# shubhamchandak94/HARC

Measured on AMD Instinct MI355X. Metric: Mreads/s reorder+encode, 100 bp, higher is better.
Workload: dtype u64 (2-bit packed bases, XOR+popcount)

## Files before the change

harc_amd/csrc/internal.h:

```cpp
#pragma once
#include <hip/hip_runtime.h>
#include <stdint.h>
#include <stdio.h>
#include <string.h>
#include <map>
#include <string>
#include <utility>
#include <vector>
#include "../../include/harc_amd.h"

#define HARC_NONE 0xFFFFFFFFu
#define HARC_MAXW 8
#define HARC_MAXW3 12
#define HARC_MAXK (1u << 20)
#define HARC_LOOK_CHUNKS 16
#ifndef HARC_NSUGG
#define HARC_NSUGG 8
#endif

void harc_set_error(const char *fmt, ...);

#define HIP_TRY(expr)                                                                                          \
    do {                                                                                                       \
        hipError_t _e = (expr);                                                                                \
// ... 67 lines not shown
    std::vector<PoolChunk> pool;
    size_t pool_cur = 0, pool_total = 0;

    uint32_t N = 0;  uint64_t *d_reads = nullptr;
    uint32_t NN = 0; uint64_t *d_nreads3 = nullptr;
    struct InBuf { void *p = nullptr; size_t cap = 0; };
    InBuf own_reads, own_nreads3;
    uint32_t N_own = 0, NN_own = 0;
    uint64_t nrec_own = 0;
    struct HarcComm *comm = nullptr;
    InBuf x_reads, x_nreads3, x_gid, x_ngid;
    uint32_t *d_gid = nullptr, *d_ngid = nullptr;
    int s2_world = 1, s2_rank = 0;
    bool s2_part = false; int s2_e0 = 0, s2_e1 = 0;
    bool replicated = false;
    uint64_t shard_info[8] = { 0, 0, 0, 0, 0, 0, 0, 0 };
    bool have_s1 = false;
    uint32_t M = 0, S = 0;
    uint32_t *d_order = nullptr; uint8_t *d_flag = nullptr, *d_pos = nullptr, *d_rc = nullptr; uint32_t *d_order_s = nullptr;
    uint64_t *d_oreads = nullptr;
    uint64_t *d_sreads = nullptr;
    bool s1_from_files = false;
    bool have_s2 = false;
    uint32_t *d_s2_order = nullptr, *d_s2_orderN = nullptr; size_t n_s2_order = 0, n_s2_orderN = 0;

    struct OutBuf { const uint8_t *ptr = nullptr; size_t len = 0; std::vector<uint8_t> own; };
    std::map<std::pair<int, int>, OutBuf> out;
    struct HostChunk { char *base; size_t size, used; };
    std::vector<HostChunk> harena;
    harc_amd_counters C;
    uint64_t digest[4] = { 0, 0, 0, 0 }; bool have_digest = false;

    char *feed_ring = nullptr; size_t feed_ring_bytes = 0;

    void *d_tmp = nullptr; size_t tmp_bytes = 0;
};

struct HarcComm {
    int world = 1, rank = 0;
    virtual ~HarcComm() {}
    virtual int allgather_u64(harc_amd_ctx *c, const uint64_t *in, int n, uint64_t *out) = 0;
    virtual int alltoallv(harc_amd_ctx *c, int narr, const void *const *send, const size_t *const *soff, const size_t *const *sbytes,
                          void *const *recv, const size_t *const *roff, const size_t *const *rbytes) = 0;
    virtual int allreduce_min_u64(harc_amd_ctx *c, unsigned long long *d_buf, size_t n) = 0;
    virtual int wait(harc_amd_ctx *c, const char *what) = 0;
    virtual const char *name() const = 0;
};
int harc_in_reserve(harc_amd_ctx *c, harc_amd_ctx::InBuf *b, size_t bytes);
void harc_reset_shard(harc_amd_ctx *c);
void harc_drop_results(harc_amd_ctx *c);

int harc_dev_alloc(harc_amd_ctx *c, void **p, size_t bytes);
void harc_dev_free(harc_amd_ctx *c, void *p);
template <class T> static inline int dalloc(harc_amd_ctx *c, T **p, size_t n) { return harc_dev_alloc(c, (void **)p, n * sizeof(T) + 16); }
int harc_tmp_reserve(harc_amd_ctx *c, size_t bytes);
int harc_raw_alloc(harc_amd_ctx *c, void **p, size_t bytes);
void harc_raw_free(harc_amd_ctx *c, void *p);
typedef unsigned long long harc_mark_t;
harc_mark_t harc_pool_mark(harc_amd_ctx *c);
void harc_pool_release(harc_amd_ctx *c, harc_mark_t m);
struct PoolScope {
    harc_amd_ctx *c; harc_mark_t mk; bool armed = true;
    explicit PoolScope(harc_amd_ctx *c_) : c(c_), mk(harc_pool_mark(c_)) {}
    PoolScope(const PoolScope &) = delete;
    PoolScope &operator=(const PoolScope &) = delete;
    ~PoolScope() { if (armed) harc_pool_release(c, mk); }
    void keep() { armed = false; }
    void release_now() { if (armed) { harc_pool_release(c, mk); armed = false; } }
};

int prim_sort_pairs_u64_u32(harc_amd_ctx *c, const uint64_t *kin, uint64_t *kout, const uint32_t *vin, uint32_t *vout, size_t n, unsigned end_bit);
#define BL_TILE_WORDS 16384u
#define BL_PART_BITS 20
#define harc_bitmap_tiles(nwords) ((uint32_t)(((uint64_t)(nwords) + BL_TILE_WORDS - 1) / BL_TILE_WORDS))
#define harc_bitmap_item(w, b0, b1) (((uint64_t)((((uint32_t)(w) % BL_TILE_WORDS) << 10) | ((uint32_t)(b0) << 5) | (uint32_t)(b1)) << BL_PART_BITS) | (uint64_t)((uint32_t)(w) / BL_TILE_WORDS))
int harc_bitmap_from_items(harc_amd_ctx *c, const uint64_t *items, uint64_t *tmp, size_t n, uint64_t nwords, uint32_t *bitmap);
int prim_sort_keys_u64(harc_amd_ctx *c, const uint64_t *kin, uint64_t *kout, size_t n, unsigned end_bit);
int prim_excl_scan_u32(harc_amd_ctx *c, const uint32_t *in, uint32_t *out, size_t n);
int prim_excl_scan_u32_to_u64(harc_amd_ctx *c, const uint32_t *in, uint64_t *out, size_t n);
int prim_excl_scan_u8_to_u64(harc_amd_ctx *c, const uint8_t *in, uint64_t *out, size_t n);
int prim_incl_scan_u64(harc_amd_ctx *c, const uint64_t *in, uint64_t *out, size_t n);
int prim_incl_max_u32(harc_amd_ctx *c, const uint32_t *in, uint32_t *out, size_t n);
int prim_incl_max_u64(harc_amd_ctx *c, const uint64_t *in, uint64_t *out, size_t n);

int s1_pack_ascii(harc_amd_ctx *c, const char *d_ascii, uint32_t n, uint32_t stride, uint64_t *d_out);
int s1_pack3_ascii(harc_amd_ctx *c, const char *d_ascii, uint32_t n, uint32_t stride, uint64_t *d_out);
int s1_unpack_to_ascii(harc_amd_ctx *c, const uint64_t *d_reads, uint32_t n, char *d_out);
int s1_bucket_reads(harc_amd_ctx *c, const uint64_t *d_packed, uint32_t n, uint32_t nb, uint32_t *d_out);
int s1_partition_reads(harc_amd_ctx *c, const uint64_t *d_packed, uint32_t n, uint32_t nb, uint64_t *d_out, unsigned long long *d_counts);
int shard_partition(harc_amd_ctx *c, const uint64_t *d_words, uint32_t n, int nwords, bool three_bit, uint32_t nb, uint32_t gid0,
                    uint64_t *d_out, uint32_t *d_gid_out, unsigned long long *d_counts);
int shard_map_ids(harc_amd_ctx *c, uint32_t *d_v, uint64_t n, const uint32_t *d_map, uint32_t nmap, unsigned int *d_err);
int stage1_run(harc_amd_ctx *c);
int stage1_make_oriented(harc_amd_ctx *c, uint32_t i0 = 0, uint32_t i1 = 0xFFFFFFFFu);
int s1_orient(harc_amd_ctx *c, const uint64_t *reads, const uint32_t *order, const uint8_t *rc, uint32_t m, uint64_t *out);
int harc_dict_alloc(harc_amd_ctx *c, DictDev *d, uint32_t n, uint64_t cap_like);
int harc_dict_build(harc_amd_ctx *c, DictDev *d, uint64_t *keys, uint32_t *ids, uint32_t n, unsigned kbits);
void harc_dict_free(harc_amd_ctx *c, DictDev *d);
int stage2_run(harc_amd_ctx *c);
int pack_order_run(harc_amd_ctx *c);

static inline std::vector<uint8_t> &out_buf(harc_amd_ctx *c, int id, int shard) { harc_amd_ctx::OutBuf &o = c->out[std::make_pair(id, shard)]; o.ptr = nullptr; o.len = 0; return o.own; }
static inline void out_slice(harc_amd_ctx *c, int id, int shard, const void *p, size_t n) { harc_amd_ctx::OutBuf &o = c->out[std::make_pair(id, shard)]; o.own.clear(); o.ptr = (const uint8_t *)p; o.len = n; }
int harc_host_alloc(harc_amd_ctx *c, void **p, size_t bytes);
void harc_host_reset(harc_amd_ctx *c);
int harc_d2h(harc_amd_ctx *c, std::vector<uint8_t> &dst, const void *d_src, size_t bytes);

int build_line_index(harc_amd_ctx *c, const char *d_txt, uint64_t nbytes, const uint64_t **nls_out, uint64_t *total_lines_out);

struct BgzfCand { uint64_t off; uint32_t bsize, hdr, isize, crc; };
struct BgzfMember { uint64_t cdata, text; uint32_t clen, isize, crc, hdr; };
struct BgzfPlan { std::vector<BgzfMember> m; uint64_t text = 0, next = 0; };
int harc_bgzf_plan(harc_amd_ctx *c, const uint8_t *d_in, uint64_t n, uint64_t start, uint64_t own_end, uint64_t base_off, BgzfPlan *plan);
int harc_bgzf_run(harc_amd_ctx *c, const uint8_t *d_in, const BgzfPlan &plan, uint64_t base_off, char *d_out);

struct BgzfOutStats { uint64_t text = 0, bytes = 0, members = 0, stored = 0; double seconds = 0; };
int harc_bgzf_deflate(harc_amd_ctx *c, const char *d_text, uint64_t n_bytes, int32_t flags, uint8_t *d_out, uint64_t out_capacity, uint64_t *n_out, BgzfOutStats *st);
```

harc_amd/csrc/prims.hip:

```cpp
#include "devutil.h"
#include <rocprim/rocprim.hpp>

int harc_tmp_reserve(harc_amd_ctx *c, size_t bytes)
{
    if (bytes <= c->tmp_bytes) return HARC_AMD_OK;
    if (c->d_tmp) harc_raw_free(c, c->d_tmp);
    c->d_tmp = nullptr; c->tmp_bytes = 0;
    size_t want = bytes + (bytes >> 3) + 4096;
    RC_TRY(harc_raw_alloc(c, &c->d_tmp, want));
    c->tmp_bytes = want;
    return HARC_AMD_OK;
}

#define PRIM_CALL(call_with_tmp)                                \
    do {                                                        \
        size_t bytes = 0; void *tmp = nullptr;                  \
        HIP_TRY(call_with_tmp);                                 \
        RC_TRY(harc_tmp_reserve(c, bytes));                     \
        tmp = c->d_tmp; bytes = c->tmp_bytes;                   \
        HIP_TRY(call_with_tmp);                                 \
    } while (0)

int prim_sort_pairs_u64_u32(harc_amd_ctx *c, const uint64_t *kin, uint64_t *kout, const uint32_t *vin, uint32_t *vout, size_t n, unsigned end_bit)
{
    if (n == 0) return HARC_AMD_OK;
    if (end_bit > 64) end_bit = 64;
    PRIM_CALL(rocprim::radix_sort_pairs(tmp, bytes, kin, kout, vin, vout, n, 0u, end_bit, c->stream));
    return HARC_AMD_OK;
}

int prim_sort_keys_u64(harc_amd_ctx *c, const uint64_t *kin, uint64_t *kout, size_t n, unsigned end_bit)
{
    if (n == 0) return HARC_AMD_OK;
    if (end_bit > 64) end_bit = 64;
    if (end_bit < 1) end_bit = 1;
    PRIM_CALL(rocprim::radix_sort_keys(tmp, bytes, kin, kout, n, 0u, end_bit, c->stream));
    return HARC_AMD_OK;
}

int prim_excl_scan_u32(harc_amd_ctx *c, const uint32_t *in, uint32_t *out, size_t n)
{
    if (n == 0) return HARC_AMD_OK;
    PRIM_CALL(rocprim::exclusive_scan(tmp, bytes, in, out, 0u, n, rocprim::plus<uint32_t>(), c->stream));
    return HARC_AMD_OK;
}

struct u32_to_u64 { __host__ __device__ uint64_t operator()(uint32_t x) const { return (uint64_t)x; } };
struct u8_to_u64 { __host__ __device__ uint64_t operator()(uint8_t x) const { return (uint64_t)x; } };

int prim_excl_scan_u32_to_u64(harc_amd_ctx *c, const uint32_t *in, uint64_t *out, size_t n)
{
    if (n == 0) return HARC_AMD_OK;
    auto it = rocprim::make_transform_iterator(in, u32_to_u64());
    PRIM_CALL(rocprim::exclusive_scan(tmp, bytes, it, out, (uint64_t)0, n, rocprim::plus<uint64_t>(), c->stream));
    return HARC_AMD_OK;
}

int prim_excl_scan_u8_to_u64(harc_amd_ctx *c, const uint8_t *in, uint64_t *out, size_t n)
{
    if (n == 0) return HARC_AMD_OK;
    auto it = rocprim::make_transform_iterator(in, u8_to_u64());
    PRIM_CALL(rocprim::exclusive_scan(tmp, bytes, it, out, (uint64_t)0, n, rocprim::plus<uint64_t>(), c->stream));
    return HARC_AMD_OK;
}

int prim_incl_scan_u64(harc_amd_ctx *c, const uint64_t *in, uint64_t *out, size_t n)
{
    if (n == 0) return HARC_AMD_OK;
    PRIM_CALL(rocprim::inclusive_scan(tmp, bytes, in, out, n, rocprim::plus<uint64_t>(), c->stream));
    return HARC_AMD_OK;
}

int prim_incl_max_u32(harc_amd_ctx *c, const uint32_t *in, uint32_t *out, size_t n)
{
    if (n == 0) return HARC_AMD_OK;
    PRIM_CALL(rocprim::inclusive_scan(tmp, bytes, in, out, n, rocprim::maximum<uint32_t>(), c->stream));
    return HARC_AMD_OK;
}

int prim_incl_max_u64(harc_amd_ctx *c, const uint64_t *in, uint64_t *out, size_t n)
{
    if (n == 0) return HARC_AMD_OK;
    PRIM_CALL(rocprim::inclusive_scan(tmp, bytes, in, out, n, rocprim::maximum<uint64_t>(), c->stream));
    return HARC_AMD_OK;
}

__global__ void k_selftest_grid(uint64_t n, unsigned long long *out)
{
    const uint64_t i = harc_gid();
    unsigned long long one = i < n ? 1ULL : 0ULL, idx = i < n ? (unsigned long long)i : 0ULL;
    for (int o = 32; o > 0; o >>= 1) { one += __shfl_xor(one, o, 64); idx += __shfl_xor(idx, o, 64); }
    if ((threadIdx.x & 63) == 0 && one) { atomicAdd(&out[0], one); atomicAdd(&out[1], idx); }
}
__global__ void k_selftest_grid32(uint32_t n, unsigned long long *out)
{
    const uint32_t i = harc_gid32();
    unsigned long long one = i < n ? 1ULL : 0ULL, idx = i < n ? (unsigned long long)i : 0ULL;
    for (int o = 32; o > 0; o >>= 1) { one += __shfl_xor(one, o, 64); idx += __shfl_xor(idx, o, 64); }
    if ((threadIdx.x & 63) == 0 && one) { atomicAdd(&out[0], one); atomicAdd(&out[1], idx); }
}
__global__ void k_selftest_fold(uint64_t n, unsigned long long *out)
{
    const uint64_t wave = harc_bid() * 4 + (threadIdx.x >> 6);
    const int lane = threadIdx.x & 63;
    const uint64_t i = wave * 16 + (uint64_t)(lane >> 2);
    const bool mine = i < n && (lane & 3) == 0;
    unsigned long long one = mine ? 1ULL : 0ULL, idx = mine ? (unsigned long long)i : 0ULL;
    for (int o = 32; o > 0; o >>= 1) { one += __shfl_xor(one, o, 64); idx += __shfl_xor(idx, o, 64); }
    if (lane == 0 && one) { atomicAdd(&out[0], one); atomicAdd(&out[1], idx); }
}
extern "C" int harc_amd_selftest_launch(harc_amd_ctx *c, uint64_t n, uint64_t *visited, uint64_t *index_sum)
{
    if (!c || !visited || !index_sum) return HARC_AMD_EINVAL;
    HIP_TRY(hipSetDevice(c->P.device));
    unsigned long long *d = nullptr, h[6] = { 0, 0, 0, 0, 0, 0 };
    HIP_TRY(hipMalloc((void **)&d, sizeof h));
    const bool n32 = n <= 0xFFFFFFFFull;
    hipError_t e = hipMemsetAsync(d, 0, sizeof h, c->stream);
    if (e == hipSuccess) { hipLaunchKernelGGL(k_selftest_grid, harc_grid256(n), dim3(256), 0, c->stream, n, d); e = hipGetLastError(); }
    if (e == hipSuccess && n32) { hipLaunchKernelGGL(k_selftest_grid32, harc_grid256(n), dim3(256), 0, c->stream, (uint32_t)n, d + 2); e = hipGetLastError(); }
    if (e == hipSuccess) { hipLaunchKernelGGL(k_selftest_fold, harc_fold256((n + 63) / 64), dim3(256), 0, c->stream, n, d + 4); e = hipGetLastError(); }
    if (e == hipSuccess) e = hipMemcpyAsync(h, d, sizeof h, hipMemcpyDeviceToHost, c->stream);
    if (e == hipSuccess) e = hipStreamSynchronize(c->stream);
    (void)hipFree(d);
    if (e != hipSuccess) { harc_set_error("harc_amd_selftest_launch: %s", hipGetErrorString(e)); return HARC_AMD_ENODEVICE; }
    int k = 0;
    if (n32 && (h[2] != h[0] || h[3] != h[1])) k = 2;
    else if (h[4] != h[0] || h[5] != h[1]) k = 4;
    if (k) harc_set_error("harc_amd_selftest_launch: %s visited %llu items (index sum %llx), the thread-per-item grid %llu (%llx)", k == 2 ? "harc_gid32" : "harc_fold256 / harc_bid", h[k], h[k + 1], h[0], h[1]);
    *visited = h[k]; *index_sum = h[k + 1];
    return k ? HARC_AMD_EINTERNAL : HARC_AMD_OK;
}
```

harc_amd/csrc/stage1.hip:

```cpp
#include "devutil.h"
#include <stdlib.h>
#include <type_traits>

struct S1Args {
    int L, maxmatch, thresh, maxsearch, Lp;
    int ds[2], de[2], kbits[2];
    uint32_t N, K;
    const uint64_t *reads;
    HashSlot *slots[2];
    uint64_t cap[2];
    const uint32_t *ids[2];
    int firstmax;
    const uint32_t *bloom[2]; uint32_t bloom_lines; int bloom_nwin[2]; uint32_t bloom_mmask;
    const uint2 *largetab;
    uint64_t *mirror;
    unsigned long long *claimed;
    uint32_t *bid;
    ChainHdr *hdr;
    uint4 *cnt;
    uint2 *steps;
    uint8_t *need;
    uint32_t *seedbuf;
    uint32_t *needrank;
    uint32_t *rmeta;
// ... 169 lines not shown
    const uint32_t i = (uint32_t)(gid / W); const int w = (int)(gid % W);
    out[gid] = reads[(size_t)idx[i] * W + w];
}
int s1_partition_reads(harc_amd_ctx *c, const uint64_t *d_packed, uint32_t n, uint32_t nb, uint64_t *d_out, unsigned long long *d_counts)
{
    HIP_TRY(hipMemsetAsync(d_counts, 0, (size_t)nb * 8, c->stream));
    if (!n) { HIP_TRY(hipStreamSynchronize(c->stream)); return HARC_AMD_OK; }
    PoolScope scope(c);
    uint32_t *b = nullptr, *i0 = nullptr, *i1 = nullptr; uint64_t *k0 = nullptr, *k1 = nullptr;
    RC_TRY(dalloc(c, &b, n)); RC_TRY(dalloc(c, &i0, n)); RC_TRY(dalloc(c, &i1, n)); RC_TRY(dalloc(c, &k0, n)); RC_TRY(dalloc(c, &k1, n));
    hipLaunchKernelGGL(k_bucket, harc_grid256(n), dim3(256), 0, c->stream, d_packed, n, c->P.readlen, c->W, nb, b);
    hipLaunchKernelGGL(k_bucket_keys, harc_grid256(n), dim3(256), 0, c->stream, (const uint32_t *)b, n, k0, i0, d_counts);
    unsigned bits = 1; while ((1u << bits) < nb) bits++;
    RC_TRY(prim_sort_pairs_u64_u32(c, k0, k1, i0, i1, n, bits));
    hipLaunchKernelGGL(k_gather_reads, harc_grid256((uint64_t)n * c->W), dim3(256), 0, c->stream, d_packed, (const uint32_t *)i1, n, c->W, d_out);
    HIP_TRY(hipGetLastError());
    HIP_TRY(hipStreamSynchronize(c->stream));
    return HARC_AMD_OK;
}

template <int W> __global__ void k_keygen2(const uint64_t *reads, uint32_t n, int off0, int nbits0, int off1, int nbits1, uint64_t *keys0, uint64_t *keys1, uint32_t *ids)
{
    const uint32_t i = harc_gid32();
    if (i >= n) return;
    uint64_t r[W];
#pragma unroll
    for (int w = 0; w < W; w++) r[w] = reads[(size_t)i * W + w];
    {
        const int wi = off0 >> 6, sh = off0 & 63;
        const uint64_t lo = sel0<W>(r, wi), hi = sel0<W>(r, wi + 1);
        uint64_t v = sh ? ((lo >> sh) | (hi << (64 - sh))) : lo;
        if (nbits0 < 64) v &= ((uint64_t)1 << nbits0) - 1;
        keys0[i] = v;
    }
    {
        const int wi = off1 >> 6, sh = off1 & 63;
        const uint64_t lo = sel0<W>(r, wi), hi = sel0<W>(r, wi + 1);
        uint64_t v = sh ? ((lo >> sh) | (hi << (64 - sh))) : lo;
        if (nbits1 < 64) v &= ((uint64_t)1 << nbits1) - 1;
        keys1[i] = v;
    }
    ids[i] = i;
}
__global__ void k_large_sizes(const unsigned long long *list, uint32_t nlist, HashSlot *s0, HashSlot *s1, uint32_t *sz)
{
    const uint32_t b = harc_gid32();
    if (b >= nlist) return;
    const unsigned long long e = list[b];
    const HashSlot *slot = ((e & 1) ? s1 : s0) + (e >> 1);
    sz[b] = slot->count & SLOT_CNT_MASK;
}
template <int W> __global__ __launch_bounds__(64) void k_large_fill(const unsigned long long *list, uint32_t nlist, HashSlot *s0, HashSlot *s1, const uint32_t *ids0, const uint32_t *ids1,
                                                                   const uint64_t *moff, const uint64_t *reads, uint2 *largetab, uint64_t *mirror)
{
    const uint32_t b = blockIdx.y * gridDim.x + blockIdx.x;
    if (b >= nlist) return;
    const int lane = threadIdx.x;
    const unsigned long long e = list[b];
    const int l = (int)(e & 1);
    HashSlot *slot = (l ? s1 : s0) + (e >> 1);
    const uint32_t st = slot->start, cnt = slot->count & SLOT_CNT_MASK;
    const uint32_t *ids = (l ? ids1 : ids0) + st;
    const uint64_t m0 = moff[b];
    for (uint32_t k = lane; k < cnt; k += 64) {
        const uint32_t rid = ids[k];
#pragma unroll
        for (int w = 0; w < W; w++) mirror[(m0 + k) * W + w] = reads[(size_t)rid * W + w];
    }
    if (lane == 0) { largetab[b] = make_uint2(st, (uint32_t)m0); slot->start = b; }
}
__global__ void k_mark_heads(const uint64_t *skeys, uint32_t n, uint32_t *head)
{
    const uint32_t i = harc_gid32();
    if (i >= n) return;
    head[i] = (i == 0 || skeys[i] != skeys[i - 1]) ? 1u : 0u;
}
__global__ void k_bin_starts(const uint32_t *head, const uint32_t *binidx, uint32_t n, uint32_t *binstart, uint32_t *nbins, const uint64_t *skeys, uint64_t cap, uint64_t *v)
{
    const uint32_t i = harc_gid32();
    if (i >= n) return;
    if (head[i]) { const uint32_t b = binidx[i]; binstart[b] = i; v[b] = bucket_slot(skeys[i], cap) + (uint64_t)n - (uint64_t)b; }
    if (i == n - 1) *nbins = binidx[i] + head[i];
}
#define HARC_LARGEBIN 16u
#define HARC_STEP_CAP 12
#define HARC_BO_FREE 1u
#define HARC_BO_CAP 3u
#define HARC_SCAN_BUDGET 12
#define MIXED_MAX (1u << 20)
#define MIXED_BUDGET 200000u
__device__ __forceinline__ uint64_t rotl64(uint64_t x, unsigned r) { r &= 63u; return r ? (x << r) | (x >> (64u - r)) : x; }
__global__ void k_mixed_find(const uint64_t *rk, uint32_t n, unsigned sbits, uint64_t *sk, uint32_t *list, unsigned int *meta)
{
    const uint32_t i = harc_gid32();
    if (i >= n) return;
    const int shift = (int)(64u - sbits);
    const uint64_t b = rotl64(rk[i], 64u - sbits);
    sk[i] = b;
    if (i == 0) return;
    const uint64_t a = rotl64(rk[i - 1], 64u - sbits);
    if (a != b && (a >> shift) == (b >> shift)) { const unsigned int at = atomicAdd(&meta[0], 1u); if (at < MIXED_MAX) list[at] = i; else meta[1] = 1u; }
}
__global__ void k_mixed_own(const uint64_t *sk, int shift, uint32_t *list, unsigned int *meta)
{
    const uint32_t t = harc_gid32();
    const unsigned int nl = meta[0] < MIXED_MAX ? meta[0] : MIXED_MAX;
    if (t >= nl || meta[1]) return;
    const uint32_t i = list[t];
    const uint64_t top = sk[i] >> shift;
    for (uint32_t h = i; h > 0 && (sk[h - 1] >> shift) == top;) {
        h--;
        if (h > 0 && sk[h] != sk[h - 1] && (sk[h - 1] >> shift) == top) { list[t] = HARC_NONE; return; }
        if (i - h > MIXED_BUDGET) { meta[1] = 1u; return; }
    }
}
__global__ void k_mixed_fix(uint64_t *sk, uint32_t *ids, uint32_t n, int shift, const uint32_t *list, unsigned int *meta)
{
    const uint32_t t = harc_gid32();
    const unsigned int nl = meta[0] < MIXED_MAX ? meta[0] : MIXED_MAX;
    if (t >= nl || meta[1]) return;
    const uint32_t i = list[t];
    if (i == HARC_NONE) return;
    const uint64_t top = sk[i] >> shift;
    uint32_t h = i;
    while (h > 0 && (sk[h - 1] >> shift) == top) h--;
    uint32_t e = i + 1;
    while (e < n && (sk[e] >> shift) == top) { e++; if (e - h > MIXED_BUDGET) { meta[1] = 1u; return; } }
    uint32_t moves = 0;
    for (uint32_t x = h + 1; x < e; x++) {
        const uint64_t kx = sk[x]; const uint32_t vx = ids[x];
        uint32_t y = x;
        while (y > h && sk[y - 1] > kx) { sk[y] = sk[y - 1]; ids[y] = ids[y - 1]; y--; if (++moves > MIXED_BUDGET) { meta[1] = 1u; return; } }
        if (y != x) { sk[y] = kx; ids[y] = vx; }
    }
}
__global__ void k_scramble_keys(uint64_t *keys, uint32_t n, unsigned rot)
{
    const uint32_t i = harc_gid32();
    if (i < n) keys[i] = rotl64(key_scramble(keys[i]), rot);
}
__global__ void k_rotate_keys(uint64_t *keys, uint32_t n, unsigned rot)
{
    const uint32_t i = harc_gid32();
    if (i < n) keys[i] = rotl64(keys[i], rot);
}
#ifndef TP_SPAN
#define TP_SPAN 1280u
#endif
__global__ __launch_bounds__(256) void k_table_place(const uint64_t *skeys, const uint32_t *sids, const uint32_t *binstart, uint32_t nbins, uint32_t n, const uint64_t *q,
                              HashSlot *slots, uint64_t cap, uint32_t bigthresh,
                              unsigned long long *large_list, unsigned int *large_n, uint32_t large_max, uint32_t large_tag, uint32_t *nbins_p, int pass, uint32_t first_block, int fill)
{
    __shared__ uint4 tile[TP_SPAN];
    if (blockIdx.x < first_block) return;
    const uint32_t i = harc_gid32();
    const bool have = i < nbins;
    auto slot_of = [&](uint32_t k) -> uint64_t { return q[k] - (uint64_t)n + (uint64_t)k; };
    const uint32_t b0 = blockIdx.x * blockDim.x, b1 = b0 + blockDim.x < nbins ? b0 + blockDim.x : nbins;
    bool tiled = false; uint64_t lo = 0, hi = 0;
    if (pass == 0 && fill && b0 < nbins) {
        lo = b0 ? slot_of(b0 - 1) + 1 : 0;
        const uint64_t last = slot_of(b1 - 1);
        if (lo < cap) {
            hi = (last >= cap || b1 == nbins || slot_of(b1) >= cap) ? cap : last + 1;
            tiled = hi - lo <= TP_SPAN;
        }
// ... 1964 lines not shown
    np = wave_sum_u32(np); nc = wave_sum_u32(nc); nu = wave_sum_u32(nu); um = wave_sum_u32(um); cf = wave_sum_u32(cf); ncs = wave_sum_u32(ncs);
    cnc = wave_sum_u32(cnc); cnu = wave_sum_u32(cnu); cncs = wave_sum_u32(cncs); sd = wave_sum_u32(sd); sc = wave_sum_u32(sc);
    if ((threadIdx.x & 63) == 0) {
        if (um) atomicAdd(&stats[ST_UNMATCHED], (unsigned long long)um);
        if (cf) atomicAdd(&stats[ST_CONFLICTS], (unsigned long long)cf);
        if (np) atomicAdd(&stats[ST_PROBES], (unsigned long long)np);
        if (nc) atomicAdd(&stats[ST_CANDS], (unsigned long long)nc);
        if (nu) atomicAdd(&stats[ST_USEFUL], (unsigned long long)nu);
        if (ncs) atomicAdd(&stats[ST_CANDS_SEQ], (unsigned long long)ncs);
        if (cnc) atomicAdd(&stats[ST_COOP_CANDS], (unsigned long long)cnc);
        if (cnu) atomicAdd(&stats[ST_COOP_USEFUL], (unsigned long long)cnu);
        if (cncs) atomicAdd(&stats[ST_COOP_CANDS_SEQ], (unsigned long long)cncs);
        if (sd) atomicAdd(&stats[ST_DENSE_STEPS], (unsigned long long)sd);
        if (sc) atomicAdd(&stats[ST_COOP_STEPS], (unsigned long long)sc);
    }
}
__global__ __launch_bounds__(256) void k_s1_singles(const uint2 *slog, unsigned long long nlog, uint32_t K, const uint32_t *base_sing, uint32_t *order_s, unsigned long long *found)
{
    __shared__ unsigned int cnt;
    if (threadIdx.x == 0) cnt = 0;
    __syncthreads();
    unsigned int mine = 0;
    for (unsigned long long i = (unsigned long long)blockIdx.x * blockDim.x + threadIdx.x; i < nlog; i += (unsigned long long)gridDim.x * blockDim.x) {
        const uint2 r = slog[i];
        if (r.x < K) { order_s[base_sing[r.x] + r.y] = (uint32_t)i; mine++; }
    }
    mine = wave_sum_u32(mine);
    if ((threadIdx.x & 63) == 0 && mine) atomicAdd(&cnt, mine);
    __syncthreads();
    if (threadIdx.x == 0 && cnt) atomicAdd(found, (unsigned long long)cnt);
}
__global__ __launch_bounds__(256) void k_pages_out(const uint2 *pg_rec, const uint2 *pg_hdr, uint32_t npages, const uint32_t *n_main, const uint32_t *base_main,
                                                   uint32_t *order, uint8_t *flag, uint8_t *pos, uint8_t *rc)
{
    const uint32_t p = blockIdx.x * 4 + (threadIdx.x >> 6), lane = threadIdx.x & 63;
    if (p >= npages) return;
    const uint2 hd = pg_hdr[p];
    const uint32_t nm = n_main[hd.x], first = hd.y * 64u;
    if (first + lane >= nm) return;
    const uint2 r = pg_rec[(size_t)p * 64 + lane];
    const size_t at = (size_t)base_main[hd.x] + first + lane;
    order[at] = r.x; pos[at] = (uint8_t)(r.y & 0xFF);
    flag[at] = (r.y >> 8) & 1 ? '1' : '0'; rc[at] = (r.y >> 9) & 1 ? 'r' : 'd';
}
template <int W> __global__ void k_orient(const uint64_t *reads, const uint32_t *order, const uint8_t *rc, uint32_t m, int L, uint64_t *out)
{
    constexpr int RPW = 64 / W;
    const int lane = threadIdx.x & 63, rl = lane / W, w = lane % W;
    const uint64_t wave = harc_gid() >> 6;
    const uint64_t i64 = wave * RPW + (uint64_t)rl;
    const uint32_t i = (uint32_t)i64;
    const bool on = rl < RPW && i64 < m;
    uint64_t mine = 0; bool rev = false;
    if (on) {
        const uint32_t rid = order[i];
        mine = reads[(size_t)rid * W + w];
        rev = rc != nullptr && rc[i] == 'r';
    }
    uint64_t r[W], o[W];
#pragma unroll
    for (int k = 0; k < W; k++) r[k] = shfl_u64(mine, rl * W + k);
    if (!on) return;
    uint64_t ow = mine;
    if (rev) { rc_words<W>(r, L, o); ow = sel0<W>(o, w); }
    out[(size_t)i * W + w] = ow;
}

int harc_dict_alloc(harc_amd_ctx *c, DictDev *d, uint32_t n, uint64_t cap_like)
{
    d->cap = 0; d->slots = nullptr; d->ids = nullptr; d->d_nbins = nullptr;
    if (n == 0) return HARC_AMD_OK;
    if (cap_like) d->cap = cap_like;
    else {
        unsigned long long m = 4;
        size_t fr = 0, tot = 0;
        if (hipMemGetInfo(&fr, &tot) == hipSuccess) { fr += c->pool_total; while (m > 2 && ((double)m * n * sizeof(HashSlot) > 0.2 * (double)fr || (double)m * n * sizeof(HashSlot) > 0.15 * (double)tot)) m--; }
        if (c->P.table_slots_per_read >= 2 && c->P.table_slots_per_read <= 4) m = (unsigned long long)c->P.table_slots_per_read;
        if (const char *e = getenv("HARC_AMD_CAPMULT")) m = strtoull(e, nullptr, 10);
        d->cap = (((m < 2 ? 2 : m) * n + 4) + 3) & ~3ull;
    }
    RC_TRY(dalloc(c, &d->slots, d->cap)); RC_TRY(dalloc(c, &d->ids, n)); RC_TRY(dalloc(c, &d->d_nbins, 2));
    return HARC_AMD_OK;
}
int harc_dict_build(harc_amd_ctx *c, DictDev *d, uint64_t *keys, uint32_t *ids, uint32_t n, unsigned kbits)
{
    (void)kbits;
    if (n == 0) return HARC_AMD_OK;
    PoolScope scope(c);
    uint64_t *k1 = nullptr; uint32_t *h0 = nullptr, *b0 = nullptr, *bs = nullptr;
    RC_TRY(dalloc(c, &k1, n)); RC_TRY(dalloc(c, &h0, n)); RC_TRY(dalloc(c, &b0, n)); RC_TRY(dalloc(c, &bs, n));
    unsigned sbits = 64;
    { unsigned lg = 1; while (((uint64_t)1 << lg) < n) lg++; sbits = ((lg + 8 + 7) / 8) * 8; if (sbits > 64) sbits = 64; }
    if (const char *e = getenv("HARC_AMD_SORT_BITS")) { const int x = atoi(e); if (x >= 1 && x <= 64) sbits = (unsigned)x; }
    uint32_t *mixed = nullptr; unsigned int *mmeta = nullptr; uint64_t *k2 = nullptr;
    RC_TRY(dalloc(c, &mixed, MIXED_MAX)); RC_TRY(dalloc(c, &mmeta, 4));
    RC_TRY(dalloc(c, &k2, n));
    uint64_t *const k2v = k2;
    hipLaunchKernelGGL(k_scramble_keys, harc_grid256(n), dim3(256), 0, c->stream, keys, n, sbits < 64 ? sbits : 0u);
    uint32_t nbins = 0;
    for (;;) {
        HIP_TRY(hipMemsetAsync(mmeta, 0, 16, c->stream));
        HIP_TRY(hipMemsetAsync(d->d_nbins, 0, 8, c->stream));
        if (sbits < 64) {
            RC_TRY(prim_sort_pairs_u64_u32(c, keys, k2, ids, d->ids, n, sbits));
            hipLaunchKernelGGL(k_mixed_find, harc_grid256(n), dim3(256), 0, c->stream, (const uint64_t *)k2, n, sbits, k1, mixed, mmeta);
            hipLaunchKernelGGL(k_mixed_own, dim3(MIXED_MAX / 256), dim3(256), 0, c->stream, (const uint64_t *)k1, (int)(64 - sbits), mixed, mmeta);
            hipLaunchKernelGGL(k_mixed_fix, dim3(MIXED_MAX / 256), dim3(256), 0, c->stream, k1, d->ids, n, (int)(64 - sbits), (const uint32_t *)mixed, mmeta);
        } else RC_TRY(prim_sort_pairs_u64_u32(c, keys, k1, ids, d->ids, n, 64));
        hipLaunchKernelGGL(k_mark_heads, harc_grid256(n), dim3(256), 0, c->stream, k1, n, h0);
        RC_TRY(prim_excl_scan_u32(c, h0, b0, n));
        hipLaunchKernelGGL(k_bin_starts, harc_grid256(n), dim3(256), 0, c->stream, h0, b0, n, bs, d->d_nbins, (const uint64_t *)k1, d->cap, k2v);
        unsigned int mm[2] = { 0, 0 };
        HIP_TRY(hipMemcpyAsync(&nbins, d->d_nbins, 4, hipMemcpyDeviceToHost, c->stream));
        HIP_TRY(hipMemcpyAsync(mm, mmeta, 8, hipMemcpyDeviceToHost, c->stream));
        HIP_TRY(hipStreamSynchronize(c->stream));
        if (getenv("HARC_AMD_TRACE")) fprintf(stderr, "[index] sort on the top %u bits: %u places where different keys share them%s\n", sbits, mm[0], mm[1] ? " -- too many or too long, sorting on all bits" : "");
        if (!mm[1] || sbits == 64) break;
        hipLaunchKernelGGL(k_rotate_keys, harc_grid256(n), dim3(256), 0, c->stream, keys, n, 64u - sbits);
        sbits = 64;
    }
    const int fill = getenv("HARC_AMD_TABLE_FILL") ? atoi(getenv("HARC_AMD_TABLE_FILL")) != 0 : (uint64_t)nbins * 16 >= d->cap;
    if (!fill) HIP_TRY(hipMemsetAsync(d->slots, 0, d->cap * sizeof(HashSlot), c->stream));
    d->nbins = nbins;
    {
        uint64_t *v = k2v, *q = keys;
        const unsigned gb = (nbins + 255) / 256;
        RC_TRY(prim_incl_max_u64(c, v, q, nbins));
        for (int pass = 0; pass < 2; pass++)
            hipLaunchKernelGGL(k_table_place, dim3(gb), dim3(256), 0, c->stream, (const uint64_t *)k1, (const uint32_t *)d->ids, (const uint32_t *)bs, nbins, n, (const uint64_t *)q,
                               d->slots, d->cap, d->bigthresh, d->large_list, d->large_n, d->large_max, d->large_tag, d->d_nbins, pass, pass == 0 ? 0u : (gb > 64 ? gb - 64 : 0u), fill);
    }
    HIP_TRY(hipGetLastError());
    uint32_t nb2[2] = { 0, 0 };
    HIP_TRY(hipMemcpyAsync(nb2, d->d_nbins, 8, hipMemcpyDeviceToHost, c->stream));
    HIP_TRY(hipStreamSynchronize(c->stream));
    scope.release_now();
    if (nb2[1]) { harc_set_error("dictionary: %u bins hold more than %u reads with the same k-mer (count field of the slot), or lie more than 16384 bins beyond the end of the table", nb2[1], SLOT_CNT_MASK); return HARC_AMD_EINVAL; }
    return HARC_AMD_OK;
}
void harc_dict_free(harc_amd_ctx *c, DictDev *d)
{
    if (d->slots) harc_dev_free(c, d->slots);
    if (d->ids) harc_dev_free(c, d->ids);
    if (d->d_nbins) harc_dev_free(c, d->d_nbins);
    d->slots = nullptr; d->ids = nullptr; d->d_nbins = nullptr; d->cap = 0;
}

static std::vector<uint16_t> make_probe_table(const harc_amd_params &P)
{
    std::vector<uint16_t> t;
    for (int j = 0; j < P.maxmatch; j++) {
        for (int l = 0; l < 2; l++) if (P.dict_end[l] + j < P.readlen) t.push_back((uint16_t)(j | (0 << 8) | (l << 9)));
        for (int l = 0; l < 2; l++) if (P.dict_start[l] > j) t.push_back((uint16_t)(j | (1 << 8) | (l << 9)));
    }
    return t;
}

static uint32_t auto_chains(uint32_t N, int reads_per_chain)
{
    uint32_t k = N / (uint32_t)(reads_per_chain > 0 ? reads_per_chain : 2048);
    const uint32_t floor_k = N / 1024 < 2048 ? N / 1024 : 2048;
    if (k < floor_k) k = floor_k;
    if (k > 65536) k = 65536;
    if (k < 1) k = 1;
    return k;
}

struct EventRing {
    static constexpr int RING = 64;
    hipEvent_t ring[RING][2];
    int ring_used = 0; uint64_t ring_next = 0; double ms = 0; uint64_t launches = 0;
    EventRing() { for (int i = 0; i < RING; i++) ring[i][0] = ring[i][1] = nullptr; }
    ~EventRing() { for (int i = 0; i < ring_used; i++) { (void)hipEventDestroy(ring[i][0]); (void)hipEventDestroy(ring[i][1]); } }
    int next_pair(hipEvent_t **pair)
    {
        const int k = (int)(ring_next % RING);
        if (k >= ring_used) { HIP_TRY(hipEventCreate(&ring[k][0])); HIP_TRY(hipEventCreate(&ring[k][1])); ring_used = k + 1; }
        else RC_TRY(collect(k));
        ring_next++; launches++;
        *pair = ring[k];
        return HARC_AMD_OK;
    }
    int collect(int k) { float x = 0; HIP_TRY(hipEventSynchronize(ring[k][1])); HIP_TRY(hipEventElapsedTime(&x, ring[k][0], ring[k][1])); ms += x; return HARC_AMD_OK; }
    int collect_all() { const uint64_t n = ring_next < (uint64_t)RING ? ring_next : (uint64_t)RING; for (uint64_t i = 0; i < n; i++) RC_TRY(collect((int)i)); ring_next = 0; return HARC_AMD_OK; }
};
struct S1Resources {
    hipEvent_t e[3] = { nullptr, nullptr, nullptr };
    hipEvent_t eb[2] = { nullptr, nullptr };
    EventRing dense, coop;
    unsigned long long *h_stats = nullptr;
    ~S1Resources()
    {
        for (hipEvent_t x : e) if (x) (void)hipEventDestroy(x);
        for (hipEvent_t x : eb) if (x) (void)hipEventDestroy(x);
        if (h_stats) (void)hipHostFree(h_stats);
    }
    int init()
    {
        for (auto &x : e) HIP_TRY(hipEventCreate(&x));
        for (auto &x : eb) HIP_TRY(hipEventCreate(&x));
        HIP_TRY(hipHostMalloc((void **)&h_stats, (ST_N + HARC_COOPCNT + 8 + 1) * 8));
        return HARC_AMD_OK;
    }
};

template <int W> static int stage1_run_w(harc_amd_ctx *c)
{
    const harc_amd_params &P = c->P;
    const uint32_t N = c->N;
    uint32_t K = P.num_chains > 0 ? (uint32_t)P.num_chains : auto_chains(N, P.reads_per_chain);
// ... 471 lines not shown
```

Measured before the change: 694.4.

## Fuse head marking, bin scan, bin starts and max-scan into one segmented scan

```diff
diff --git a/harc_amd/csrc/idx_scan.h b/harc_amd/csrc/idx_scan.h
--- /dev/null
+++ b/harc_amd/csrc/idx_scan.h
@@ -0,0 +1,40 @@
+#pragma once
+#include <stdint.h>
+
+#if defined(__HIPCC__)
+#define IX_HD __host__ __device__ __forceinline__
+#else
+#define IX_HD static inline
+#endif
+
+#define IDX_SCAN_TILE 2048u
+
+struct IdxSeg { uint32_t c; uint32_t head; uint64_t m; };
+
+IX_HD uint64_t ix_bucket_slot(uint64_t h, uint64_t cap)
+{
+    const uint64_t nb = cap >> 2;
+    if (nb >> 32) {
+#if defined(__HIP_DEVICE_COMPILE__)
+        return __umul64hi(h, nb) << 2;
+#else
+        return (uint64_t)(((unsigned __int128)h * nb) >> 64) << 2;
+#endif
+    }
+    return (((h >> 32) * (uint64_t)(uint32_t)nb) >> 32) << 2;
+}
+IX_HD IdxSeg ix_lift(uint64_t key, int opens, uint64_t cap, uint32_t n)
+{
+    IdxSeg r;
+    r.c = opens ? 1u : 0u; r.head = r.c;
+    r.m = opens ? ix_bucket_slot(key, cap) + (uint64_t)n : 0;
+    return r;
+}
+IX_HD IdxSeg ix_combine(IdxSeg a, IdxSeg b)
+{
+    const uint64_t mb = b.m ? b.m - (uint64_t)a.c : 0;
+    IdxSeg r;
+    r.c = a.c + b.c; r.head = b.head;
+    r.m = a.m > mb ? a.m : mb;
+    return r;
+}
diff --git a/harc_amd/csrc/internal.h b/harc_amd/csrc/internal.h
--- a/harc_amd/csrc/internal.h
+++ b/harc_amd/csrc/internal.h
@@ -173,6 +173,7 @@
 int prim_incl_scan_u64(harc_amd_ctx *c, const uint64_t *in, uint64_t *out, size_t n);
 int prim_incl_max_u32(harc_amd_ctx *c, const uint32_t *in, uint32_t *out, size_t n);
 int prim_incl_max_u64(harc_amd_ctx *c, const uint64_t *in, uint64_t *out, size_t n);
+int prim_index_scan(harc_amd_ctx *c, const uint64_t *skeys, uint32_t n, uint64_t cap, uint32_t *bs, uint64_t *q, uint32_t *nbins);
 
 int s1_pack_ascii(harc_amd_ctx *c, const char *d_ascii, uint32_t n, uint32_t stride, uint64_t *d_out);
 int s1_pack3_ascii(harc_amd_ctx *c, const char *d_ascii, uint32_t n, uint32_t stride, uint64_t *d_out);
diff --git a/harc_amd/csrc/prims.hip b/harc_amd/csrc/prims.hip
--- a/harc_amd/csrc/prims.hip
+++ b/harc_amd/csrc/prims.hip
@@ -1,4 +1,5 @@
 #include "devutil.h"
+#include "idx_scan.h"
 #include <rocprim/rocprim.hpp>
 
 int harc_tmp_reserve(harc_amd_ctx *c, size_t bytes)
@@ -85,6 +86,39 @@
     return HARC_AMD_OK;
 }
 
+struct IxLift {
+    const uint64_t *k; uint64_t cap; uint32_t n;
+    __host__ __device__ IdxSeg operator()(size_t i) const { const uint64_t a = k[i]; return ix_lift(a, i == 0 || k[i - 1] != a, cap, n); }
+};
+struct IxPlus { __host__ __device__ IdxSeg operator()(const IdxSeg &a, const IdxSeg &b) const { return ix_combine(a, b); } };
+struct IxOutRef {
+    uint32_t *bs; uint64_t *q; uint32_t *nbins; uint32_t n; size_t i;
+    __host__ __device__ const IxOutRef &operator=(const IdxSeg &v) const
+    {
+        if (v.head) { bs[v.c - 1] = (uint32_t)i; q[v.c - 1] = v.m; }
+        if (i + 1 == (size_t)n) *nbins = v.c;
+        return *this;
+    }
+};
+struct IxOut {
+    using iterator_category = std::random_access_iterator_tag; using value_type = IdxSeg; using difference_type = std::ptrdiff_t; using pointer = IdxSeg *; using reference = IxOutRef;
+    uint32_t *bs; uint64_t *q; uint32_t *nbins; uint32_t n; size_t i;
+    __host__ __device__ IxOutRef operator[](size_t j) const { return IxOutRef{ bs, q, nbins, n, i + j }; }
+    __host__ __device__ IxOutRef operator*() const { return IxOutRef{ bs, q, nbins, n, i }; }
+    __host__ __device__ IxOut operator+(size_t j) const { return IxOut{ bs, q, nbins, n, i + j }; }
+};
+int prim_index_scan(harc_amd_ctx *c, const uint64_t *skeys, uint32_t n, uint64_t cap, uint32_t *bs, uint64_t *q, uint32_t *nbins)
+{
+    if (n == 0) return HARC_AMD_OK;
+    static_assert(IDX_SCAN_TILE == 256u * 8u, "idx_scan.h names the tile of this configuration");
+    using cfg = rocprim::scan_config<256, IDX_SCAN_TILE / 256u, rocprim::block_load_method::block_load_transpose, rocprim::block_store_method::block_store_transpose,
+                                     rocprim::block_scan_algorithm::using_warp_scan>;
+    auto in = rocprim::make_transform_iterator(rocprim::counting_iterator<size_t>(0), IxLift{ skeys, cap, n });
+    IxOut out{ bs, q, nbins, n, 0 };
+    PRIM_CALL(rocprim::inclusive_scan<cfg>(tmp, bytes, in, out, (size_t)n, IxPlus(), c->stream));
+    return HARC_AMD_OK;
+}
+
 __global__ void k_selftest_grid(uint64_t n, unsigned long long *out)
 {
     const uint64_t i = harc_gid();
diff --git a/harc_amd/csrc/stage1.hip b/harc_amd/csrc/stage1.hip
--- a/harc_amd/csrc/stage1.hip
+++ b/harc_amd/csrc/stage1.hip
@@ -275,6 +275,15 @@
     if (head[i]) { const uint32_t b = binidx[i]; binstart[b] = i; v[b] = bucket_slot(skeys[i], cap) + (uint64_t)n - (uint64_t)b; }
     if (i == n - 1) *nbins = binidx[i] + head[i];
 }
+__global__ void k_dict_diff(const uint32_t *bs, const uint32_t *bsr, const uint64_t *q, const uint64_t *qr, uint32_t nbins, const uint32_t *nbins_ref, unsigned long long *ndiff)
+{
+    const uint32_t b = harc_gid32();
+    if (b > nbins) return;
+    unsigned int bad;
+    if (b == nbins) bad = *nbins_ref != nbins;
+    else bad = (unsigned int)(bs[b] != bsr[b]) + (unsigned int)(q[b] != qr[b]);
+    if (bad) atomicAdd(ndiff, (unsigned long long)bad);
+}
 #define HARC_LARGEBIN 16u
 #define HARC_STEP_CAP 12
 #define HARC_BO_FREE 1u
@@ -2405,20 +2414,31 @@
     RC_TRY(dalloc(c, &d->slots, d->cap)); RC_TRY(dalloc(c, &d->ids, n)); RC_TRY(dalloc(c, &d->d_nbins, 2));
     return HARC_AMD_OK;
 }
+static unsigned harc_dict_sort_bits(uint32_t n)
+{
+    unsigned sbits = 64;
+    { unsigned lg = 1; while (((uint64_t)1 << lg) < n) lg++; sbits = ((lg + 8 + 7) / 8) * 8; if (sbits > 64) sbits = 64; }
+    if (const char *e = getenv("HARC_AMD_SORT_BITS")) { const int x = atoi(e); if (x >= 1 && x <= 64) sbits = (unsigned)x; }
+    return sbits;
+}
 int harc_dict_build(harc_amd_ctx *c, DictDev *d, uint64_t *keys, uint32_t *ids, uint32_t n, unsigned kbits)
 {
     (void)kbits;
     if (n == 0) return HARC_AMD_OK;
     PoolScope scope(c);
-    uint64_t *k1 = nullptr; uint32_t *h0 = nullptr, *b0 = nullptr, *bs = nullptr;
-    RC_TRY(dalloc(c, &k1, n)); RC_TRY(dalloc(c, &h0, n)); RC_TRY(dalloc(c, &b0, n)); RC_TRY(dalloc(c, &bs, n));
-    unsigned sbits = 64;
-    { unsigned lg = 1; while (((uint64_t)1 << lg) < n) lg++; sbits = ((lg + 8 + 7) / 8) * 8; if (sbits > 64) sbits = 64; }
-    if (const char *e = getenv("HARC_AMD_SORT_BITS")) { const int x = atoi(e); if (x >= 1 && x <= 64) sbits = (unsigned)x; }
+    uint64_t *k1 = nullptr; uint32_t *bs = nullptr;
+    RC_TRY(dalloc(c, &k1, n)); RC_TRY(dalloc(c, &bs, n));
+    const bool dverify = getenv("HARC_AMD_DICT_VERIFY") != nullptr;
+    uint32_t *h0 = nullptr, *b0 = nullptr, *bsr = nullptr, *nbr = nullptr; uint64_t *vr = nullptr, *qr = nullptr; unsigned long long *ndiff = nullptr;
+    if (dverify) {
+        RC_TRY(dalloc(c, &h0, n)); RC_TRY(dalloc(c, &b0, n)); RC_TRY(dalloc(c, &bsr, n)); RC_TRY(dalloc(c, &nbr, 2));
+        RC_TRY(dalloc(c, &vr, n)); RC_TRY(dalloc(c, &qr, n)); RC_TRY(dalloc(c, &ndiff, 1));
+    }
+    unsigned sbits = harc_dict_sort_bits(n);
     uint32_t *mixed = nullptr; unsigned int *mmeta = nullptr; uint64_t *k2 = nullptr;
     RC_TRY(dalloc(c, &mixed, MIXED_MAX)); RC_TRY(dalloc(c, &mmeta, 4));
     RC_TRY(dalloc(c, &k2, n));
-    uint64_t *const k2v = k2;
+    uint64_t *const q = k2;
     hipLaunchKernelGGL(k_scramble_keys, harc_grid256(n), dim3(256), 0, c->stream, keys, n, sbits < 64 ? sbits : 0u);
     uint32_t nbins = 0;
     for (;;) {
@@ -2430,9 +2450,7 @@
             hipLaunchKernelGGL(k_mixed_own, dim3(MIXED_MAX / 256), dim3(256), 0, c->stream, (const uint64_t *)k1, (int)(64 - sbits), mixed, mmeta);
             hipLaunchKernelGGL(k_mixed_fix, dim3(MIXED_MAX / 256), dim3(256), 0, c->stream, k1, d->ids, n, (int)(64 - sbits), (const uint32_t *)mixed, mmeta);
         } else RC_TRY(prim_sort_pairs_u64_u32(c, keys, k1, ids, d->ids, n, 64));
-        hipLaunchKernelGGL(k_mark_heads, harc_grid256(n), dim3(256), 0, c->stream, k1, n, h0);
-        RC_TRY(prim_excl_scan_u32(c, h0, b0, n));
-        hipLaunchKernelGGL(k_bin_starts, harc_grid256(n), dim3(256), 0, c->stream, h0, b0, n, bs, d->d_nbins, (const uint64_t *)k1, d->cap, k2v);
+        RC_TRY(prim_index_scan(c, k1, n, d->cap, bs, q, d->d_nbins));
         unsigned int mm[2] = { 0, 0 };
         HIP_TRY(hipMemcpyAsync(&nbins, d->d_nbins, 4, hipMemcpyDeviceToHost, c->stream));
         HIP_TRY(hipMemcpyAsync(mm, mmeta, 8, hipMemcpyDeviceToHost, c->stream));
@@ -2442,13 +2460,25 @@
         hipLaunchKernelGGL(k_rotate_keys, harc_grid256(n), dim3(256), 0, c->stream, keys, n, 64u - sbits);
         sbits = 64;
     }
+    if (nbins == 0 || nbins > n) { harc_set_error("dictionary: the scan over %u sorted keys counts %u bins", n, nbins); return HARC_AMD_EINTERNAL; }
     const int fill = getenv("HARC_AMD_TABLE_FILL") ? atoi(getenv("HARC_AMD_TABLE_FILL")) != 0 : (uint64_t)nbins * 16 >= d->cap;
     if (!fill) HIP_TRY(hipMemsetAsync(d->slots, 0, d->cap * sizeof(HashSlot), c->stream));
     d->nbins = nbins;
+    if (dverify) {
+        unsigned long long hnd = 0;
+        HIP_TRY(hipMemsetAsync(nbr, 0, 8, c->stream)); HIP_TRY(hipMemsetAsync(ndiff, 0, 8, c->stream));
+        hipLaunchKernelGGL(k_mark_heads, harc_grid256(n), dim3(256), 0, c->stream, k1, n, h0);
+        RC_TRY(prim_excl_scan_u32(c, h0, b0, n));
+        hipLaunchKernelGGL(k_bin_starts, harc_grid256(n), dim3(256), 0, c->stream, h0, b0, n, bsr, nbr, (const uint64_t *)k1, d->cap, vr);
+        RC_TRY(prim_incl_max_u64(c, vr, qr, nbins));
+        hipLaunchKernelGGL(k_dict_diff, harc_grid256((uint64_t)nbins + 1), dim3(256), 0, c->stream, (const uint32_t *)bs, (const uint32_t *)bsr, (const uint64_t *)q, (const uint64_t *)qr,
+                           nbins, (const uint32_t *)nbr, ndiff);
+        HIP_TRY(hipMemcpyAsync(&hnd, ndiff, 8, hipMemcpyDeviceToHost, c->stream));
+        HIP_TRY(hipStreamSynchronize(c->stream));
+        if (hnd) { harc_set_error("dictionary: the one-pass scan differs from the four reference launches in %llu words of bs, q and nbins", hnd); return HARC_AMD_EINTERNAL; }
+    }
     {
-        uint64_t *v = k2v, *q = keys;
         const unsigned gb = (nbins + 255) / 256;
-        RC_TRY(prim_incl_max_u64(c, v, q, nbins));
         for (int pass = 0; pass < 2; pass++)
             hipLaunchKernelGGL(k_table_place, dim3(gb), dim3(256), 0, c->stream, (const uint64_t *)k1, (const uint32_t *)d->ids, (const uint32_t *)bs, nbins, n, (const uint64_t *)q,
                                d->slots, d->cap, d->bigthresh, d->large_list, d->large_n, d->large_max, d->large_tag, d->d_nbins, pass, pass == 0 ? 0u : (gb > 64 ? gb - 64 : 0u), fill);
```

Result: no change. 695.7, median of 6 (+0.2%).
